# riveSunder/therldaisyworld

Measured on AMD Instinct MI355X. Metric: cell-updates/sec (grid x batch), fused stencil+growth step, higher is better.
Workload: dtype f32

## Files before the change

### therldaisyworld_amd/csrc/dw_api.hip

```cpp
#include <hip/hip_runtime.h>

#include <cmath>
#include <cstdarg>
#include <cstdio>
#include <cstdlib>
#include <cstring>
#include <memory>
#include <new>
#include <type_traits>
#include <vector>

#include "../../include/daisyworld_hip.h"
#include "dw_kernels.hpp"
#include "dw_host_util.hpp"
#include "dw_plan.hpp"
#include "dw_series.hpp"

using namespace dw;

static thread_local char g_err[512] = "";

static int fail(int code, const char* fmt, ...) {
    va_list ap;
    va_start(ap, fmt);
// ... 489 lines not shown
template <class F>
static auto with_fused_layout(const StepPlan& pl, F&& f) {
    if (pl.packed) return f(int_c<kFusedRot>{}, std::true_type{});
    return with_int<kFusedRot, kFusedRing, kFusedOvl>(pl.fused_mode, [&](auto MODE) { return f(MODE, std::false_type{}); });
}

static int launch_forward_fused2(dw_handle* h, double L1, double L2, unsigned int* pstats = nullptr,
                                 float thr_hi = 0.f, StatsDev* trace = nullptr) {
    const dw_params& p = h->prm;
    const StepPlan& pl = h->plan;
    const bool exact = p.precision == DW_PRECISION_EXACT;
    PhysF32 P1, P2;
    if (exact) derive_f32_pair(p, L1, L2, &P1, &P2);
    else { P1 = derive_f32(p, L1); P2 = derive_f32(p, L2); }
    const StepOut o = step_out(h);
    const FusedGeom& g = pl.fgeom;
    const dim3 grid((unsigned)g.chunk * 8u);
    const plane_t *inL = h->L16[h->cur].get(), *inD = h->D16[h->cur].get();
    auto exact_args = [&] {
        return FusedExactArgs{inL, inD, o.L, o.D, g, P1, lum_part(P2), o.zero_me, o.zero_n, pstats, thr_hi, make_f64(p, L1), L1, L2};
    };
    if (trace && exact) {
        const TraceExactArgs A{exact_args(), trace, h->sw.force_rescan ? 1 : 0};
        with_int<kFusedRot, kFusedOvl>(pl.fused_mode, [&](auto MODE) {
            with_bool(pl.sym_albedo, [&](auto SYM) {
                hipLaunchKernelGGL((trace_pair_exact<MODE, SYM>), grid, dim3(256), 0, h->stream, A);
            });
        });
    } else if (trace) {
        with_int<kFusedRot, kFusedOvl>(pl.fused_mode, [&](auto MODE) {
            hipLaunchKernelGGL((trace_pair_fast<MODE>), grid, dim3(256), 0, h->stream, inL, inD, o.L, o.D, g, P1, P2, o.zero_me,
                               o.zero_n, trace);
        });
    } else if (pl.fmt_planes && !pstats && !exact) {
        hipLaunchKernelGGL((step_stream_fused2_fmt_pw<kFusedOvl>), grid, dim3(256), 0, h->stream, inL, inD, o.L, o.D, g, P1, P2,
                           o.zero_me, o.zero_n);
    } else if (exact) {
        const FusedExactArgs A = exact_args();
        with_bool(pstats != nullptr, [&](auto STATS) {
            with_fused_layout(pl, [&](auto MODE, auto PACK) {
                with_bool(pl.sym_albedo, [&](auto SYM) {
                    hipLaunchKernelGGL((step_stream_fused2_exact<MODE, PACK, STATS, SYM>), grid, dim3(256), 0, h->stream, A);
                });
            });
        });
    } else {
        with_bool(pstats != nullptr, [&](auto STATS) {
            with_fused_layout(pl, [&](auto MODE, auto PACK) {
                hipLaunchKernelGGL((step_stream_fused2<MODE, PACK, STATS>), grid, dim3(256), 0, h->stream, inL, inD, o.L, o.D, g,
                                   P1, P2, o.zero_me, o.zero_n, pstats, thr_hi);
            });
        });
    }
    HIPCHK(hipGetLastError());
    step_done(h, L2, false);
    return DW_OK;
}

static int launch_agents(dw_handle* h, const int* d_action, int act_b, int act_n, bool standalone = false,
                         double* d_reward = nullptr, unsigned char* d_done = nullptr, unsigned char* d_ok = nullptr) {
    const dw_params& p = h->prm;
    if (p.n_agents == 0) return DW_OK;
    NEED(h->have_state, DW_ESTATE, "no state uploaded");
    NEED(h->have_agents, DW_ESTATE, "no agents uploaded (call dw_upload_agents or dw_init_random)");
    NEED(p.collision_mode == 0 || standalone, DW_EINVAL,
         "collision_mode=1: call dw_update_agents, apply the collision pass (it consumes the caller's RNG) to the "
// ... 1712 lines not shown
    HIPCHK(hipEventSynchronize(h->ev1));
    HIPCHK(hipEventElapsedTime(elapsed_ms, h->ev0, h->ev1));
    return DW_OK;
}

int dw_device_planes(dw_handle* h, int which, void** light, void** dark) {
    NEED(h && light && dark, DW_EINVAL, "null argument");
    NEED(which == DW_STATE_CURRENT || which == DW_STATE_PREVIOUS, DW_EINVAL, "bad state selector");
    const int buf = which == DW_STATE_CURRENT ? h->cur : 1 - h->cur;
    NEED(which != DW_STATE_CURRENT || cur_quantised(h), DW_ESTATE,
         "the current state is an un-quantised upload: it has no binary16 planes before the first step");
    *light = h->L16[buf].get();
    *dark = h->D16[buf].get();
    return DW_OK;
}

int dw_kernel_info(dw_handle* h, char* buf, size_t buflen) {
    NEED(h && buf && buflen, DW_EINVAL, "null argument");
    const dw_params& p = h->prm;
    const StepPlan& pl = h->plan;
    const char* prec = p.precision == DW_PRECISION_EXACT ? "exact" : (p.precision == DW_PRECISION_FAST ? "fast" : "f64");
    static const char* const halo_name[] = {"rotate", "dpp-old", "general", "packed"};
    if (pl.kind == STEP_STREAM) {
        const StripGeom& g = pl.sgeom;
        snprintf(buf, buflen,
                 "step_stream_%s<halo=%s> wave-strip=%dx256 cells, register window + DPP neighbours, %d-row blocks in "
                 "flight%s, %d strips, grid=%d x 256 threads (4 strips each), XCD-chunked",
                 prec, halo_name[pl.halo], g.SR,
                 p.precision == DW_PRECISION_EXACT ? DW_STREAM_RB_EXACT : DW_STREAM_RB_FAST,
                 p.precision == DW_PRECISION_EXACT ? ", in-wave float64 fix-up from an LDS queue" : "", g.nstrips,
                 g.chunk * 8);
        if (pl.allow_fuse) {
            const size_t n = std::strlen(buf);
            snprintf(buf + n, buflen - n, "; dw_step_n fuses step pairs (step_stream_fused2%s%s)",
                     p.precision == DW_PRECISION_EXACT ? "_exact" : "", pl.fmt_planes ? "_fmt_pw, format buffer accesses" : "");
        }
    } else if (pl.kind == STEP_TILED) {
        const int TR = (256 / pl.tcq) * pl.rpt;
        snprintf(buf, buflen,
                 "step_tiled<TCQ=%d,RPT=%d,%s> tile=%dx%d cells, %zu B LDS/workgroup, %d tiles, grid=%d x 256 threads, "
                 "XCD-chunked",
                 pl.tcq, pl.rpt, prec, TR, pl.tcq * 4, pl.tile_lds, pl.geom.ntiles, pl.geom.chunk * 8);
    } else {
        snprintf(buf, buflen, "step_generic<%s> one thread per cell, grid=(%d,%d) x 256 threads", prec,
                 (p.height * p.width + 255) / 256, p.batch);
    }
    {
        const size_t n = std::strlen(buf);
        snprintf(buf + n, buflen - n, pl.trace_pairs ? "; trace: step pairs" : "; trace: single steps");
    }
    {
        const size_t n = std::strlen(buf);
        snprintf(buf + n, buflen - n, pl.pw_stream ? "; per-world L: wave strips" : "; per-world L: generic");
    }
    {
        static const char* const form_name[] = {"launches per step", "workgroup (LDS)", "one wave per world"};
        const size_t n = std::strlen(buf);
        snprintf(buf + n, buflen - n, "; episode: %s; mlp episode: %s", form_name[episode_form(h)], form_name[episode_mlp_form(h)]);
    }
    {
        const size_t n = std::strlen(buf);
        snprintf(buf + n, buflen - n, "; ensemble episode: %s", ensemble_episode_wave(h) ? "one wave per world" : "launches per step");
    }
    {
        const size_t n = std::strlen(buf);
        snprintf(buf + n, buflen - n, "; episode trace: %s", episode_trace_wave(h) ? "one wave per world" : "launches per step");
    }
    if (pl.first_stream) {
// ... 53 lines not shown
```

### therldaisyworld_amd/csrc/dw_common.hpp

```cpp
#pragma once
#include <type_traits>

#include "dw_physics.hpp"
#include "dw_types.hpp"

namespace dw {

__device__ __forceinline__ float wave_sum(float v) {
#pragma unroll
    for (int o = 32; o > 0; o >>= 1) v += __shfl_xor(v, o, 64);
    return v;
}
__device__ __forceinline__ float wave_max(float v) {
#pragma unroll
    for (int o = 32; o > 0; o >>= 1) v = fmaxf(v, __shfl_xor(v, o, 64));
    return v;
}

__device__ __forceinline__ double to_natural(double x) { return x; }
__device__ __forceinline__ double to_natural(float k) { return (double)k / 1000.0; }
__device__ __forceinline__ double to_natural(plane_t k) { return dw_permille_to_natural((double)(float)k); }
__device__ __forceinline__ float to_permille(double x) { return (float)(x * 1000.0); }
__device__ __forceinline__ float to_permille(float k) { return k; }
__device__ __forceinline__ float to_permille(plane_t k) { return (float)k; }

typedef _Float16 dw_f16x4 __attribute__((ext_vector_type(4)));
typedef unsigned int dw_u32x2 __attribute__((ext_vector_type(2)));
__device__ __forceinline__ dw_f16x4 stream_load4_raw(const plane_t* p) { return *reinterpret_cast<const dw_f16x4*>(p); }
__device__ __forceinline__ float4 widen4(const dw_f16x4& v) { return make_float4((float)v.x, (float)v.y, (float)v.z, (float)v.w); }
__device__ __forceinline__ float4 stream_load4(const plane_t* p) { return widen4(stream_load4_raw(p)); }
__device__ __forceinline__ void stream_store4(plane_t* p, const float4& v) {
    dw_u32x2 t;
    t.x = __builtin_bit_cast(unsigned int, __builtin_amdgcn_cvt_pkrtz(v.x, v.y));
    t.y = __builtin_bit_cast(unsigned int, __builtin_amdgcn_cvt_pkrtz(v.z, v.w));
    __builtin_nontemporal_store(t, reinterpret_cast<dw_u32x2*>(p));
}

typedef float dw_fmt_f32x4 __attribute__((ext_vector_type(4)));
typedef int dw_i32x4 __attribute__((ext_vector_type(4)));
__device__ dw_fmt_f32x4 dw_buf_load_fmt4(dw_i32x4 rsrc, int voff, int soff, int aux) __asm("llvm.amdgcn.raw.buffer.load.format.v4f32");
__device__ void dw_buf_store_fmt4(dw_fmt_f32x4 v, dw_i32x4 rsrc, int voff, int soff, int aux) __asm("llvm.amdgcn.raw.buffer.store.format.v4f32");
constexpr int kBufAuxNonTemporal = 2;
__device__ __forceinline__ dw_i32x4 fmt_plane_rsrc(const plane_t* plane, int world, unsigned int world_bytes) {
    const unsigned long long base = (unsigned long long)plane + (unsigned long long)world * world_bytes;
    dw_i32x4 r;
    r.x = __builtin_amdgcn_readfirstlane((int)(unsigned int)base);
    r.y = __builtin_amdgcn_readfirstlane((int)(unsigned int)(base >> 32)) & 0xffff;
    r.z = __builtin_amdgcn_readfirstlane((int)world_bytes);
    r.w = 0x00067FAC;
    return r;
}
__device__ __forceinline__ float4 fmt_load4(const dw_i32x4& rsrc, int voff, int soff) {
    const dw_fmt_f32x4 v = dw_buf_load_fmt4(rsrc, voff, soff, 0);
    return make_float4(v.x, v.y, v.z, v.w);
}
__device__ __forceinline__ void fmt_store4(const dw_i32x4& rsrc, int voff, int soff, const float4& v) {
    dw_buf_store_fmt4(dw_fmt_f32x4{v.x, v.y, v.z, v.w}, rsrc, voff, soff, kBufAuxNonTemporal);
}
__device__ __forceinline__ float4 widen4(const float4& v) {
    typedef float f2 __attribute__((ext_vector_type(2)));
    unsigned long long lo, hi;
    asm("v_pk_mov_b32 %0, %1, %1 op_sel:[0,1]" : "=v"(lo) : "v"(f2{v.x, v.y}));
    asm("v_pk_mov_b32 %0, %1, %1 op_sel:[0,1]" : "=v"(hi) : "v"(f2{v.z, v.w}));
    return make_float4(__uint_as_float((unsigned int)lo), __uint_as_float((unsigned int)(lo >> 32)),
                       __uint_as_float((unsigned int)hi), __uint_as_float((unsigned int)(hi >> 32)));
}

__device__ __forceinline__ int wrap_near(int v, int n) { return v < 0 ? v + n : (v >= n ? v - n : v); }
__device__ __forceinline__ int wrap_near2(int v, int n) { return wrap_near(wrap_near(v, n), n); }

template <typename T>
__device__ __forceinline__ void gather9(const T* __restrict__ plane, int H, int W, int r, int c,
                                        double out[9]) {
    const int ru = r == 0 ? H - 1 : r - 1, rd = r == H - 1 ? 0 : r + 1;
    const int cl = c == 0 ? W - 1 : c - 1, cr = c == W - 1 ? 0 : c + 1;
    const int rows[3] = {ru, r, rd}, cols[3] = {cl, c, cr};
#pragma unroll
    for (int a = 0; a < 3; ++a)
#pragma unroll
        for (int b = 0; b < 3; ++b) out[a * 3 + b] = to_natural(plane[(size_t)rows[a] * W + cols[b]]);
}

struct Row4 {
    float x[4];
    float h2[4];
};

// ... 55 lines not shown
```

### therldaisyworld_amd/csrc/dw_plan.hpp

```cpp
#pragma once
#include <climits>
#include <cmath>
#include <cstddef>
#include <cstdio>
#include <cstdlib>
#include <cstring>

#include "../../include/daisyworld_hip.h"
#include "dw_types.hpp"

namespace dw {

struct Switches {
    bool no_sym = false, no_pack = false, no_fuse = false, no_ring = false, no_fmt_planes = false, no_episode_kernel = false,
         no_episode_wave = false, no_agent_fuse = false, no_agent_preapply = false, first_f64 = false,
         first_generic = false, force_rescan = false, test_hooks = false;
    int pack_min_strips = -1, strip_rows = 0, tile_rpt = 0, queue_cap = -1, mismatch_cap = -1, trace_rows = 0;
    double first_slack = -1.0;
    char kernel[16] = {0};
    char text[256] = {0};
};
inline const char* test_hook(const char* name) {
    return std::getenv("DW_TEST_HOOKS") ? std::getenv(name) : nullptr;
}
inline Switches read_switches() {
    Switches w;
    auto note = [&](const char* name, const char* val) {
        const size_t n = std::strlen(w.text);
        snprintf(w.text + n, sizeof(w.text) - n, "%s%s%s%s", n ? " " : "", name, val ? "=" : "", val ? val : "");
    };
    auto flag = [&](const char* name, bool& dst) { if (std::getenv(name)) { dst = true; note(name, nullptr); } };
    auto num = [&](const char* name, int& dst, bool test) {
        if (const char* e = test ? test_hook(name) : std::getenv(name)) { dst = std::atoi(e); note(name, e); }
    };
    w.test_hooks = std::getenv("DW_TEST_HOOKS") != nullptr;
    flag("DW_NO_SYM", w.no_sym); flag("DW_NO_PACK", w.no_pack); flag("DW_NO_FUSE", w.no_fuse); flag("DW_NO_RING", w.no_ring);
    flag("DW_NO_FMT_PLANES", w.no_fmt_planes);
    flag("DW_NO_EPISODE_KERNEL", w.no_episode_kernel); flag("DW_NO_EPISODE_WAVE", w.no_episode_wave);
    flag("DW_NO_AGENT_FUSE", w.no_agent_fuse); flag("DW_NO_AGENT_PREAPPLY", w.no_agent_preapply);
    flag("DW_FIRST_STEP_F64", w.first_f64); flag("DW_FIRST_GENERIC", w.first_generic);
    num("DW_PACK_MIN_STRIPS", w.pack_min_strips, false); num("DW_STRIP_ROWS", w.strip_rows, false);
    num("DW_TILE_RPT", w.tile_rpt, false);
    num("DW_TEST_QUEUE_CAP", w.queue_cap, true); num("DW_TEST_MISMATCH_CAP", w.mismatch_cap, true);
    num("DW_TEST_TRACE_ROWS", w.trace_rows, true);
    if (test_hook("DW_TEST_FORCE_RESCAN")) { w.force_rescan = true; note("DW_TEST_FORCE_RESCAN", nullptr); }
    if (const char* e = test_hook("DW_TEST_FIRST_SLACK")) { w.first_slack = std::atof(e); note("DW_TEST_FIRST_SLACK", e); }
    if (const char* e = std::getenv("DW_KERNEL")) { snprintf(w.kernel, sizeof(w.kernel), "%s", e); note("DW_KERNEL", e); }
    return w;
}

inline dw_params with_world_params(dw_params p, const dw_world_params& w) {
    p.p = w.p; p.g = w.g; p.S = w.S; p.sigma = w.sigma; p.gamma = w.gamma; p.q = w.q; p.q2 = w.q2; p.dt = w.dt;
    p.albedo_bare = w.albedo_bare; p.albedo_light = w.albedo_light; p.albedo_dark = w.albedo_dark;
    p.temp_optimal = w.temp_optimal;
    return p;
}
inline dw_world_params world_params_of(const dw_params& p) {
    return dw_world_params{p.p, p.g, p.S, p.sigma, p.gamma, p.q, p.q2, p.dt, p.albedo_bare, p.albedo_light, p.albedo_dark,
                           p.temp_optimal};
}
inline bool albedo_symmetric(double bare, double light, double dark) { return (dark - bare) == -(light - bare); }
inline bool worlds_symmetric(const dw_world_params* worlds, size_t B) {
    for (size_t b = 0; b < B; ++b)
        if (!albedo_symmetric(worlds[b].albedo_bare, worlds[b].albedo_light, worlds[b].albedo_dark)) return false;
    return true;
}

inline PhysF64 make_f64(const dw_params& p, double L) {
    PhysF64 P;
    P.p = p.p; P.g = p.g; P.S = p.S; P.sigma = p.sigma; P.gamma = p.gamma; P.q = p.q; P.q2 = p.q2;
// ... 139 lines not shown
    const double kmax = 1000.0;
    const double a1 = std::fabs((double)P.a1), a2 = std::fabs((double)P.a2), a3 = std::fabs((double)P.a3), a4 = std::fabs((double)P.a4);
    const EConst c0 = e_const(p, L);
    const double c0m = std::fmax(std::fabs(c0.c0l), std::fabs(c0.c0d));
    const double Mmax = (a1 + a2) * 8 * kmax + (a3 + a4) * kmax;
    const double de_max = (8.0 * u + iota) * Mmax + u * c0m;
    const TieChain t = tie_chain(p, c0, P.a1, P.a2, P.a3, P.a4, de_max);
    const double kbe = cbeta_host(p);
    const double Dmin = kbe * (std::sqrt(std::sqrt(t.vlo)) + 1.0) * (std::sqrt(t.vlo) + 1.0);
    const double kK = 5.0 * u + iota;
    const double safety = t.safety, pu = t.pu, kbmax = t.kbmax;
    FirstStepBound B;
    B.a1 = round_up(a1); B.a2 = round_up(a2); B.a3 = round_up(a3); B.a4 = round_up(a4);
    B.c_de = round_up(safety * (8.0 * u + iota) * (1.0 + 8.0 * u));
    B.c_c0 = round_up(safety * u * c0m);
    B.eK0 = round_up(safety * (pu + (kK + 2.0 * u) * std::fabs(p.p) + kbmax * u + ((kK + 3.0 * u) + u) * std::fabs(p.gamma)));
    B.eK1 = round_up(safety * (pu + (kK + 2.0 * u) * std::fabs(p.p) + kbmax * (u + 2.0 * t.ew)));
    B.cW = round_up(safety * 2.0 * kbmax / Dmin);
    B.eA = round_up(safety * ((kK + 3.0 * u) + u + (kK + u)));
    B.cS = round_up(safety * u);
    B.slack = t.admissible ? 4e-6f : 1.0f;
    if (test_slack > (double)B.slack) B.slack = (float)test_slack;
    return B;
}

enum StepKind { STEP_GENERIC, STEP_TILED, STEP_STREAM };
struct StepPlan {
    StepKind kind = STEP_GENERIC;
    int halo = 0;
    bool packed = false;
    bool allow_fuse = false;
    int fused_mode = kFusedOvl;
    bool fmt_planes = false;
    bool trace_pairs = false;
    bool sym_albedo = false;
    int tcq = 0, rpt = 0;
    Geom geom{};
    size_t tile_lds = 0;
    StripGeom sgeom{};
    FusedGeom fgeom{};
    int first_prec = 2;
    bool first_stream = false;
    FirstGeom first_geom{};
    bool need_fixq = false;
    bool pw_stream = false;
};

inline int halo_form(int W) { return W < 256 ? 3 : (W == 256 ? 0 : (W % 256 == 0 ? 1 : 2)); }

inline int strip_rows(long groups, int H, long target) {
    int sr = 64;
    while (sr > 8 && groups * ((H + sr - 1) / sr) < target) sr >>= 1;
    return H < sr ? H : sr;
}

inline int strip_rows_or_override(const Switches& sw, int cap, long groups, int H, long target) {
    if (sw.strip_rows < 1) return strip_rows(groups, H, target);
    const int want = sw.strip_rows < cap ? sw.strip_rows : cap;
    return H < want ? H : want;
}

inline StepPlan plan_steps(const dw_params& p, const Switches& sw) {
    StepPlan s;
    s.sym_albedo = albedo_symmetric(p.albedo_bare, p.albedo_light, p.albedo_dark) && !sw.no_sym;
    s.halo = halo_form(p.width);
    const int lpw = p.width / 4, wpr = lpw ? 64 / lpw : 0;
    const bool pack_shape = p.width >= 8 && p.width < 256 && wpr >= 1 && wpr * lpw * 10 >= 64 * 7 && !sw.no_pack;
    const long pack_strips = pack_shape ? (long)((p.batch + wpr - 1) / wpr) * ((p.height + 63) / 64) : 0;
    const bool packable = pack_shape && pack_strips >= (sw.pack_min_strips >= 0 ? sw.pack_min_strips : 512);
    const bool quads = p.precision != DW_PRECISION_F64 && p.width % 4 == 0;
    if (quads && (p.width >= 256 || packable) && std::strcmp(sw.kernel, "tiled") != 0) {
        s.kind = STEP_STREAM;
        s.packed = p.width < 256;
        StripGeom& g = s.sgeom;
        g.B = p.batch; g.H = p.height; g.W = p.width;
        g.ncs = (p.width + 255) / 256;
        g.lpw = s.packed ? lpw : 64;
        g.wpr = s.packed ? wpr : 1;
        const long groups = s.packed ? (p.batch + wpr - 1) / wpr : p.batch;
        g.SR = strip_rows_or_override(sw, INT_MAX, groups * g.ncs, p.height, 2048);
        g.nrs = (p.height + g.SR - 1) / g.SR;
        g.nstrips = (int)(groups * g.nrs * g.ncs);
        g.nwg = (g.nstrips + 3) / 4;
        g.chunk = (g.nwg + 7) / 8;
        g.qcap = kWaveQueueCap;
        int mcap = kMismatchCap;
        if (sw.queue_cap >= 0 && sw.queue_cap < kWaveQueueCap) g.qcap = sw.queue_cap;
        if (sw.mismatch_cap >= 0 && sw.mismatch_cap < kMismatchCap) mcap = sw.mismatch_cap;
        g.force_rescan = sw.force_rescan ? 1 : 0;
        s.allow_fuse = !sw.no_fuse;
        const bool ring = p.width == 1024 && !sw.no_ring;
        s.fused_mode = p.width <= 256 ? kFusedRot : (ring ? kFusedRing : kFusedOvl);
        FusedGeom& f = s.fgeom;
        f.B = p.batch; f.H = p.height; f.W = p.width;
        f.SR = g.SR;
        f.nrs = g.nrs;
        f.lpw = g.lpw; f.wpr = g.wpr;
        f.cols_per_strip = p.width <= 256 ? 256 : (ring ? 1024 : 248);
        f.ncs = s.packed ? 1 : (p.width + f.cols_per_strip - 1) / f.cols_per_strip;
        f.nstrips = (int)(groups * f.nrs * f.ncs);
        f.nwg = ring ? f.nstrips : (f.nstrips + 3) / 4;
        f.chunk = (f.nwg + 7) / 8;
        f.qcap = g.qcap;
        f.mcap = mcap;
        f.sure_need = 9 * p.n_agents + 9 * mcap + 1;
        s.trace_pairs = s.allow_fuse && !s.packed && s.fused_mode != kFusedRing;
        s.fmt_planes = p.precision == DW_PRECISION_FAST && s.allow_fuse && !s.packed && s.fused_mode == kFusedOvl && !sw.no_fmt_planes &&
                       (size_t)p.height * p.width * sizeof(plane_t) < ((size_t)1 << 31);
    } else if (quads && p.width >= 64) {
        s.kind = STEP_TILED;
        const int Wq = p.width / 4;
        if (Wq >= 64) {
            s.tcq = 64; s.rpt = 4;
            if (sw.tile_rpt == 2 || sw.tile_rpt == 4 || sw.tile_rpt == 8) s.rpt = sw.tile_rpt;
        }
        else if (Wq >= 32) { s.tcq = 32; s.rpt = 4; }
        else { s.tcq = 16; s.rpt = 2; }
        const int TR = (256 / s.tcq) * s.rpt;
        Geom& g = s.geom;
        g.B = p.batch; g.H = p.height; g.W = p.width; g.Wq = Wq;
        g.tiles_r = (p.height + TR - 1) / TR;
        g.tiles_c = (Wq + s.tcq - 1) / s.tcq;
        g.ntiles = p.batch * g.tiles_r * g.tiles_c;
        g.chunk = (g.ntiles + 7) / 8;
        g.qcap = kMaxFix;
        if (sw.queue_cap >= 0 && sw.queue_cap < kMaxFix) g.qcap = sw.queue_cap;
        s.tile_lds = (size_t)2 * (TR + 2) * (s.tcq + 2) * 4 * sizeof(float);
    }
    s.need_fixq = p.precision == DW_PRECISION_EXACT && s.kind == STEP_TILED;
    s.pw_stream = s.kind == STEP_STREAM && !s.packed;
    s.first_prec = p.precision == DW_PRECISION_FAST ? 1 : (p.precision == DW_PRECISION_EXACT && !sw.first_f64 ? 3 : 2);
    s.first_stream = (p.width % 256 == 0 || s.kind == STEP_STREAM) && s.first_prec != 2 && !sw.first_generic;
    if (s.first_stream) {
        FirstGeom& fg = s.first_geom;
        fg.B = p.batch; fg.H = p.height; fg.W = p.width;
        fg.lpw = s.packed ? lpw : 64;
        fg.wpr = s.packed ? wpr : 1;
        fg.ncs = s.packed ? 1 : (p.width + 255) / 256;
        const long groups = s.packed ? (p.batch + fg.wpr - 1) / fg.wpr : p.batch;
        fg.SR = strip_rows_or_override(sw, 64, groups * fg.ncs, p.height, 4096);
        fg.nrs = (p.height + fg.SR - 1) / fg.SR;
// ... 7 lines not shown
```

### therldaisyworld_amd/csrc/dw_step_fused.hpp

```cpp
#pragma once
#include <type_traits>
#include "dw_step_stream.hpp"
#include "dw_types.hpp"

namespace dw {


template <typename TI>
__device__ inline unsigned int exact1_word(const TI* __restrict__ pL, const TI* __restrict__ pD, int H, int W,
                                           int r, int c, const PhysF64& Pa) {
    const int rr = wrap_near2(r, H), cc = wrap_near2(c, W);
    const int ru = rr == 0 ? H - 1 : rr - 1, rd = rr == H - 1 ? 0 : rr + 1;
    const int cl = cc == 0 ? W - 1 : cc - 1, cr = cc == W - 1 ? 0 : cc + 1;
    const int rows[3] = {ru, rr, rd}, cols[3] = {cl, cc, cr};
    unsigned int w1[9];
#pragma unroll
    for (int x = 0; x < 3; ++x)
#pragma unroll
        for (int y = 0; y < 3; ++y) {
            const size_t o = (size_t)rows[x] * W + cols[y];
            w1[x * 3 + y] = (unsigned)(float)pL[o] | ((unsigned)(float)pD[o] << 16);
        }
    const NewCoverF64 s1 = cell_f64_lean(Pa, w1);
    return (unsigned)dw_round3_k(s1.nl) | ((unsigned)dw_round3_k(s1.nd) << 16);
}

template <typename TI>
__device__ inline void exact2_cell(const TI* __restrict__ pL, const TI* __restrict__ pD, int H, int W, int r,
                                   int c, const PhysF64& Pa, const PhysF64& Pb, float& kl, float& kd) {
    unsigned int w2[9];
#pragma unroll
    for (int a = 0; a < 3; ++a)
#pragma unroll
        for (int e = 0; e < 3; ++e) {
            int rr = r + a - 1, cc = c + e - 1;
            rr = rr < 0 ? rr + H : (rr >= H ? rr - H : rr);
            cc = cc < 0 ? cc + W : (cc >= W ? cc - W : cc);
            const int ru = rr == 0 ? H - 1 : rr - 1, rd = rr == H - 1 ? 0 : rr + 1;
            const int cl = cc == 0 ? W - 1 : cc - 1, cr = cc == W - 1 ? 0 : cc + 1;
            const int rows[3] = {ru, rr, rd}, cols[3] = {cl, cc, cr};
            unsigned int w1[9];
#pragma unroll
            for (int x = 0; x < 3; ++x)
#pragma unroll
                for (int y = 0; y < 3; ++y) {
                    const size_t o = (size_t)rows[x] * W + cols[y];
                    w1[x * 3 + y] = (unsigned)(float)pL[o] | ((unsigned)(float)pD[o] << 16);
                }
            const NewCoverF64 s1 = cell_f64_lean(Pa, w1);
            w2[a * 3 + e] = (unsigned)dw_round3_k(s1.nl) | ((unsigned)dw_round3_k(s1.nd) << 16);
        }
    const NewCoverF64 s2 = cell_f64_lean(Pb, w2);
    kl = (float)dw_round3_k(s2.nl);
    kd = (float)dw_round3_k(s2.nd);
}

template <int MODE, bool EXACT, bool PACK = false, bool STATS = false, bool SYM = false, typename TI = plane_t,
          typename TO = plane_t, bool TRACE = false, bool FMT = false>
__device__ __forceinline__ void fused2_body(const TI* __restrict__ inL, const TI* __restrict__ inD,
                                            TO* __restrict__ outL, TO* __restrict__ outD, const FusedGeom& G,
                                            const PhysF32& P1_, const PhysF32& P2_, const PhysF64& P64,
                                            const double& La, const double& Lb,
                                            unsigned long long* __restrict__ zero_me, int zero_n,
                                            unsigned int* __restrict__ pstats = nullptr, float thr_hi = 0.f,
                                            StatsDev* __restrict__ trace = nullptr, int trace_rescan = 0) {
    constexpr bool ROT = MODE == kFusedRot, RING = MODE == kFusedRing;
    static_assert(!RING || !PACK, "the ring exchange is written for un-packed worlds");
    static_assert(!TRACE || (!PACK && !STATS && !RING), "the trace form exists for un-packed overlapped / rotating strips");
    static_assert(!FMT || (MODE == kFusedOvl && !EXACT && !PACK && !STATS && !TRACE), "the format-access form exists for the plain float32 kernel on overlapped strips");
    __shared__ float s_edge[RING ? 2 * 4 * 8 : 1];
    __shared__ uint4 s_queue[EXACT ? 4 * kWaveQueueCap * 3 : 1];
    __shared__ unsigned int s_mm[EXACT ? 4 * kMismatchCap : 1];
    const int bid = blockIdx.x;
    const int wg = (bid & 7) * G.chunk + (bid >> 3);
    if (wg >= G.nwg) return;
    const int tid = threadIdx.x, wv = tid >> 6, lane = tid & 63;
    if (wg == 0)
        for (int i = tid; i < zero_n; i += 256) zero_me[i] = 0ull;
    const int s = RING ? wg : __builtin_amdgcn_readfirstlane(wg * 4 + wv);
    if (!RING && s >= G.nstrips) return;
    uint4* q = s_queue + (EXACT ? wv * kWaveQueueCap * 3 : 0);
    unsigned int* mm = s_mm + (EXACT ? wv * kMismatchCap : 0);
    const int spw = G.nrs * G.ncs;
    const int b = s / spw;
    const int sw = s - b * spw;
    const int rs = sw / G.ncs, cs = sw - rs * G.ncs;
    const int r0 = rs * G.SR;
    const int nr = min(G.SR, G.H - r0);
    const int pw = PACK ? lane / G.lpw : 0, pj = PACK ? lane - pw * G.lpw : 0;
    const int lsrc = PACK ? (pj == 0 ? lane + G.lpw - 1 : lane - 1) : 0;
    const int rsrc = PACK ? (pj == G.lpw - 1 ? lane - (G.lpw - 1) : lane + 1) : 0;
    auto world_off = [&](int lc) -> size_t {
        return (size_t)(PACK ? min(b * G.wpr + min((lc >> 2) / G.lpw, G.wpr - 1), G.B - 1) : b) * G.H * G.W;
    };
    const size_t woff = world_off(4 * lane);
    const int c00 = ROT ? 0 : (RING ? 256 * __builtin_amdgcn_readfirstlane(wv) : cs * 248 - 4);
    int col = PACK ? 4 * pj : c00 + 4 * lane;
    col = col < 0 ? col + G.W : col;
    col = col >= G.W ? col - G.W : col;
    const bool writes = PACK ? (pw < G.wpr && b * G.wpr + pw < G.B)
                             : ((ROT || RING) ? true : (lane >= 1 && lane <= 62 && cs * 248 + 4 * (lane - 1) < G.W));
    bool need1[4] = {true, true, true, true};
    if (PACK) { need1[0] = need1[1] = need1[2] = need1[3] = writes; }
    if (EXACT && !ROT && !RING) {
        const bool wl = __builtin_amdgcn_update_dpp(0, writes ? 1 : 0, kDppWaveShr1, 0xf, 0xf, false) != 0;
        const bool wr = __builtin_amdgcn_update_dpp(0, writes ? 1 : 0, kDppWaveShl1, 0xf, 0xf, false) != 0;
        need1[0] = writes || wl;
        need1[1] = writes;
        need1[2] = writes;
        need1[3] = writes || wr;
    }
    constexpr bool LANE_BOOLS = PACK || (STATS && MODE == kFusedOvl);
    using TieT = std::conditional_t<LANE_BOOLS, bool, unsigned long long>;
    TieT need1m[4], writes_m;
    if constexpr (LANE_BOOLS) {
        for (int i = 0; i < 4; ++i) need1m[i] = need1[i];
        writes_m = writes;
    } else {
        for (int i = 0; i < 4; ++i) need1m[i] = lane_mask(need1[i]);
        writes_m = lane_mask(writes);
    }
    const TI* pL = inL + woff;
    const TI* pD = inD + woff;

    dw_i32x4 fmt_inL, fmt_inD, fmt_outL, fmt_outD;
    int fmt_col = 0, fmt_row = 0;
    if constexpr (FMT) {
        const unsigned int world_bytes = (unsigned int)(G.H * G.W) * 2u;
        fmt_inL = fmt_plane_rsrc(inL, b, world_bytes);
        fmt_inD = fmt_plane_rsrc(inD, b, world_bytes);
        fmt_outL = fmt_plane_rsrc(outL, b, world_bytes);
        fmt_outD = fmt_plane_rsrc(outD, b, world_bytes);
        fmt_col = col * 2;
        fmt_row = G.W * 2;
    }
    struct RawIn { std::conditional_t<FMT, float4, dw_f16x4> l, d; };
    auto load_raw = [&](int rr) -> RawIn {
        rr = min(rr, r0 + nr + 1);
        rr = rr < 0 ? rr + G.H : rr;
        rr = rr >= G.H ? rr - G.H : rr;
        RawIn w;
        if constexpr (FMT) {
            w.l = fmt_load4(fmt_inL, fmt_col, rr * fmt_row);
            w.d = fmt_load4(fmt_inD, fmt_col, rr * fmt_row);
        } else {
            w.l = stream_load4_raw(pL + (size_t)rr * G.W + col);
            w.d = stream_load4_raw(pD + (size_t)rr * G.W + col);
        }
        return w;
    };
    auto pin_edge_sums = [&](Row4& L, Row4& D) {
        asm volatile("" : "+v"(L.h2[0]), "+v"(L.h2[3]), "+v"(D.h2[0]), "+v"(D.h2[3]));
    };
    auto nbrs = [&](const float4& v, float& a, float& c) {
        if (PACK) { a = __shfl(v.w, lsrc, 64); c = __shfl(v.x, rsrc, 64); }
        else if (ROT) { a = dpp_mov_nb<kDppWaveRor1>(v.w); c = dpp_mov_nb<kDppWaveRol1>(v.x); }
        else { a = dpp_mov_nb<kDppWaveShr1>(v.w); c = dpp_mov_nb<kDppWaveShl1>(v.x); }
    };
    auto to_rows4 = [&](const float4& l, const float4& d, Row4& L, Row4& D) {
        float a, c;
        nbrs(l, a, c);
        L = make_row(l, a, c);
        nbrs(d, a, c);
        D = make_row(d, a, c);
    };
    int ring_par = 0;
    auto rows_ring = [&](const float4* v, Row4* const* out, auto NC) {
        constexpr int n = decltype(NC)::value;
        float* mine = s_edge + (ring_par * 4 + wv) * 8;
        if (lane == 63) {
#pragma unroll
            for (int i = 0; i < n; ++i) mine[i] = v[i].w;
        }
        if (lane == 0) {
#pragma unroll
            for (int i = 0; i < n; ++i) mine[4 + i] = v[i].x;
        }
        __syncthreads();
        const float* lw = s_edge + (ring_par * 4 + ((wv + 3) & 3)) * 8;
        const float* rw = s_edge + (ring_par * 4 + ((wv + 1) & 3)) * 8 + 4;
#pragma unroll
        for (int i = 0; i < n; ++i) {
            const float a = dpp_mov<kDppWaveShr1>(lw[i], v[i].w);
            const float c = dpp_mov<kDppWaveShl1>(rw[i], v[i].x);
            *out[i] = make_row(v[i], a, c);
        }
        ring_par ^= 1;
    };
    unsigned int nq = 0;
// ... 194 lines not shown
            Row4* const ob[2] = {&IL[2], &ID[2]};
            rows_ring(va, oa, std::integral_constant<int, 4>{});
            rows_ring(vb, ob, std::integral_constant<int, 2>{});
        } else {
            to_rows4(widen4(p0.l), widen4(p0.d), IL[0], ID[0]);
            to_rows4(widen4(p1.l), widen4(p1.d), IL[1], ID[1]);
            to_rows4(widen4(p2.l), widen4(p2.d), IL[2], ID[2]);
        }
    }
    using U0 = std::integral_constant<int, 0>;
    using U1 = std::integral_constant<int, 1>;
    using U2 = std::integral_constant<int, 2>;
    auto iter = [&](auto U, auto D1, auto D2, int j, auto ST, auto MINE) {
        constexpr int u = decltype(U)::value;
        constexpr bool do1 = decltype(D1)::value, do2 = decltype(D2)::value;
        constexpr bool st_on = STATS && decltype(ST)::value;
        RawIn nx;
        if (do1) nx = load_raw(r0 + j);
        __builtin_amdgcn_sched_barrier(0);
        float l1[4], d1[4], l2[4], d2[4];
        TieT tie1[4], tie2[4];
        float sm1 = 0.f, sm2 = 0.f;
        if (do2)
            row_cells(P2, SL[u], SL[(u + 1) % 3], SL[(u + 2) % 3], SD[u], SD[(u + 1) % 3], SD[(u + 2) % 3], l2, d2, tie2,
                      use2, st_on ? &sm2 : nullptr);
        if (do1)
            row_cells(P1, IL[(u + 2) % 3], IL[u], IL[(u + 1) % 3], ID[(u + 2) % 3], ID[u], ID[(u + 1) % 3], l1, d1, tie1,
                      need1m, st_on ? &sm1 : nullptr);
        if (do2) {
            row_queue(SL[u], SL[(u + 1) % 3], SL[(u + 2) % 3], SD[u], SD[(u + 1) % 3], SD[(u + 2) % 3], l2, d2, tie2, 2,
                      j - 2);
            if (st_on) stats_step2(sm2);
            if constexpr (TRACE) trace_step2(l2, d2);
            if constexpr (FMT) {
                if (writes) {
                    fmt_store4(fmt_outL, fmt_col, (r0 + j - 4) * fmt_row, make_float4(l2[0], l2[1], l2[2], l2[3]));
                    fmt_store4(fmt_outD, fmt_col, (r0 + j - 4) * fmt_row, make_float4(d2[0], d2[1], d2[2], d2[3]));
                }
            } else if (writes) {
                const size_t off = woff + (size_t)(r0 + j - 4) * G.W + col;
                stream_store4(outL + off, make_float4(l2[0], l2[1], l2[2], l2[3]));
                stream_store4(outD + off, make_float4(d2[0], d2[1], d2[2], d2[3]));
            }
        }
        if (do1) {
            row_queue(IL[(u + 2) % 3], IL[u], IL[(u + 1) % 3], ID[(u + 2) % 3], ID[u], ID[(u + 1) % 3], l1, d1, tie1, 1, j);
            if (st_on) stats_step1(sm1, l1, d1, tie1, j >= 2 && j <= nr + 1);
            if constexpr (TRACE) {
                if (decltype(MINE)::value || (j >= 2 && j <= nr + 1)) trace_step1(l1, d1, tie1);
            }
            if constexpr (RING) {
                const float4 v[4] = {make_float4(l1[0], l1[1], l1[2], l1[3]), make_float4(d1[0], d1[1], d1[2], d1[3]),
                                     widen4(nx.l), widen4(nx.d)};
                Row4* const o[4] = {&SL[u], &SD[u], &IL[(u + 2) % 3], &ID[(u + 2) % 3]};
                rows_ring(v, o, std::integral_constant<int, 4>{});
            } else {
                to_rows4(make_float4(l1[0], l1[1], l1[2], l1[3]), make_float4(d1[0], d1[1], d1[2], d1[3]), SL[u], SD[u]);
                __builtin_amdgcn_sched_barrier(0);
                to_rows4(widen4(nx.l), widen4(nx.d), IL[(u + 2) % 3], ID[(u + 2) % 3]);
                if (!PACK) pin_edge_sums(IL[(u + 2) % 3], ID[(u + 2) % 3]);
            }
        }
    };
    using Yes = std::true_type;
    using No = std::false_type;
    iter(U1{}, Yes{}, No{}, 1, Yes{}, No{});
    iter(U2{}, Yes{}, No{}, 2, Yes{}, No{});
// ... 236 lines not shown
        }
    }
}

#ifndef DW_FUSED_FAST_WAVES
#define DW_FUSED_FAST_WAVES 4
#endif
template <int MODE, bool PACK, bool STATS>
constexpr int fused_fast_waves() { return ((MODE == kFusedRing && STATS) || PACK) ? 3 : DW_FUSED_FAST_WAVES; }
template <int MODE, bool PACK = false, bool STATS = false>
__global__ __launch_bounds__(256)
__attribute__((amdgpu_waves_per_eu(fused_fast_waves<MODE, PACK, STATS>(), fused_fast_waves<MODE, PACK, STATS>())))
void step_stream_fused2(const plane_t* __restrict__ inL, const plane_t* __restrict__ inD,
                                                          plane_t* __restrict__ outL, plane_t* __restrict__ outD,
                                                          FusedGeom G, PhysF32 P1, PhysF32 P2,
                                                          unsigned long long* __restrict__ zero_me, int zero_n,
                                                          unsigned int* __restrict__ pstats, float thr_hi) {
    const PhysF64 dummy{};
    const double zero = 0.0;
    fused2_body<MODE, false, PACK, STATS>(inL, inD, outL, outD, G, P1, P2, dummy, zero, zero, zero_me, zero_n, pstats, thr_hi);
}

template <int MODE>
__global__ __launch_bounds__(256) __attribute__((amdgpu_waves_per_eu(DW_FUSED_FAST_WAVES, DW_FUSED_FAST_WAVES)))
void step_stream_fused2_fmt_pw(const plane_t* __restrict__ inL, const plane_t* __restrict__ inD,
                               plane_t* __restrict__ outL, plane_t* __restrict__ outD, FusedGeom G, PhysF32 P1, PhysF32 P2,
                               unsigned long long* __restrict__ zero_me, int zero_n) {
    const PhysF64 dummy{};
    const double zero = 0.0;
    fused2_body<MODE, false, false, false, false, plane_t, plane_t, false, true>(inL, inD, outL, outD, G, P1, P2, dummy, zero,
                                                                                  zero, zero_me, zero_n);
}

#ifndef DW_EXACT_PACK_WAVES
#define DW_EXACT_PACK_WAVES 3
#endif
template <int MODE, bool PACK, bool STATS>
constexpr int fused_exact_waves() {
    return (PACK && STATS) || (STATS && MODE == kFusedRing) ? 2 : (PACK ? DW_EXACT_PACK_WAVES : 3);
}
struct FusedExactArgs {
    const plane_t* inL; const plane_t* inD; plane_t* outL; plane_t* outD;
    FusedGeom G;
    PhysF32 P1; PhysLumF32 lum2;
    unsigned long long* zero_me; int zero_n;
    unsigned int* pstats; float thr_hi;
    PhysF64 P64; double La; double Lb;
};

template <int MODE, bool PACK = false, bool STATS = false, bool SYM = false>
__global__ __launch_bounds__(256)
__attribute__((amdgpu_waves_per_eu(fused_exact_waves<MODE, PACK, STATS>(), fused_exact_waves<MODE, PACK, STATS>())))
void step_stream_fused2_exact(FusedExactArgs A) {
    const FusedExactArgs& cold = kernarg_struct<FusedExactArgs>();
    const PhysF32 P2 = with_lum(A.P1, A.lum2);
    fused2_body<MODE, true, PACK, STATS, SYM>(A.inL, A.inD, A.outL, A.outD, A.G, A.P1, P2, cold.P64, cold.La, cold.Lb, A.zero_me,
                                             A.zero_n, A.pstats, A.thr_hi);
}

#ifndef DW_TRACE_FAST_WAVES
#define DW_TRACE_FAST_WAVES 3
#endif
#ifndef DW_TRACE_EXACT_WAVES
#define DW_TRACE_EXACT_WAVES 2
#endif
template <int MODE>
// ... 28 lines not shown
```

### therldaisyworld_amd/csrc/dw_types.hpp

```cpp
#pragma once

namespace dw {

typedef _Float16 plane_t;

struct PhysF64 {
    double p, g, S, sigma, gamma, q, q2, dt;
    double ab, al, ad, To;
    double L;
    double w0, w1, w2;
};

typedef float dw_f32x2 __attribute__((ext_vector_type(2)));
#define DW_PAIR(lo_name, hi_name, pair_name) \
    union { struct { float lo_name, hi_name; }; dw_f32x2 pair_name; }

struct PhysF32 {
    DW_PAIR(a1h, a2h, a12h);
    DW_PAIR(a3h, a4h, a34h);
    DW_PAIR(a1l, a2l, a12l);
    DW_PAIR(a3l, a4l, a34l);
    DW_PAIR(c0lh, c0ll, c0l);
    DW_PAIR(c0dh, dc0l, c0d);
    DW_PAIR(a1, a2, a12);
// ... 43 lines not shown

struct StripGeom {
    int B, H, W;
    int SR;
    int ncs, nrs;
    int nstrips;
    int nwg;
    int chunk;
    int qcap;
    int lpw, wpr;
    int force_rescan;
};

struct FusedGeom {
    int B, H, W;
    int SR;
    int ncs, nrs;
    int nstrips, nwg, chunk;
    int cols_per_strip;
    int qcap, mcap;
    int lpw, wpr;
    int sure_need;
};

struct FirstGeom {
    int B, H, W;
    int SR;
    int ncs, nrs;
    int nstrips;
    int lpw, wpr;
};

enum { kFusedOvl = 0, kFusedRot = 1, kFusedRing = 2 };
constexpr int kWaveQueueCap = 256;
constexpr int kMismatchCap = 64;
constexpr int kMaxFix = 1024;
constexpr int kNumQueues = 256;

}
```

Before: 787.0 billion.

## Add seam-strip layout: 252-column wave strips with wrapped lane and leftover band kernel

```diff
diff --git a/therldaisyworld_amd/csrc/dw_api.hip b/therldaisyworld_amd/csrc/dw_api.hip
--- a/therldaisyworld_amd/csrc/dw_api.hip
+++ b/therldaisyworld_amd/csrc/dw_api.hip
@@ -545,6 +545,13 @@
             hipLaunchKernelGGL((trace_pair_fast<MODE>), grid, dim3(256), 0, h->stream, inL, inD, o.L, o.D, g, P1, P2, o.zero_me,
                                o.zero_n, trace);
         });
+    } else if (pl.seam_strips && !pstats && !exact) {
+        const FusedGeom &gs = pl.seam_geom, &gl = pl.left_geom;
+        hipLaunchKernelGGL(step_stream_fused2_seam_pw, dim3((unsigned)gs.chunk * 8u), dim3(256), 0, h->stream, inL, inD, o.L, o.D,
+                           gs, P1, P2, o.zero_me, o.zero_n);
+        if (gl.nstrips)
+            hipLaunchKernelGGL(step_stream_fused2_left_pw, dim3((unsigned)gl.chunk * 8u), dim3(256), 0, h->stream, inL, inD, o.L,
+                               o.D, gl, P1, P2, o.zero_me, 0);
     } else if (pl.fmt_planes && !pstats && !exact) {
         hipLaunchKernelGGL((step_stream_fused2_fmt_pw<kFusedOvl>), grid, dim3(256), 0, h->stream, inL, inD, o.L, o.D, g, P1, P2,
                            o.zero_me, o.zero_n);
@@ -2323,8 +2330,16 @@
                  g.chunk * 8);
         if (pl.allow_fuse) {
             const size_t n = std::strlen(buf);
-            snprintf(buf + n, buflen - n, "; dw_step_n fuses step pairs (step_stream_fused2%s%s)",
-                     p.precision == DW_PRECISION_EXACT ? "_exact" : "", pl.fmt_planes ? "_fmt_pw, format buffer accesses" : "");
+            snprintf(buf + n, buflen - n, "; dw_step_n fuses step pairs (step_stream_fused2%s%s",
+                     p.precision == DW_PRECISION_EXACT ? "_exact" : "",
+                     pl.seam_strips ? "_seam_pw, format buffer accesses" : (pl.fmt_planes ? "_fmt_pw, format buffer accesses" : ""));
+            if (pl.seam_strips) {
+                const size_t m = std::strlen(buf);
+                snprintf(buf + m, buflen - m, ", seam strips: %d x %d columns + %d columns of %d row bands per wave", pl.seam_geom.ncs,
+                         kSeamCols, pl.left_geom.cols_per_strip, pl.left_geom.wpr);
+            }
+            const size_t m = std::strlen(buf);
+            snprintf(buf + m, buflen - m, ")");
         }
     } else if (pl.kind == STEP_TILED) {
         const int TR = (256 / pl.tcq) * pl.rpt;
diff --git a/therldaisyworld_amd/csrc/dw_common.hpp b/therldaisyworld_amd/csrc/dw_common.hpp
--- a/therldaisyworld_amd/csrc/dw_common.hpp
+++ b/therldaisyworld_amd/csrc/dw_common.hpp
@@ -39,20 +39,27 @@
 typedef float dw_fmt_f32x4 __attribute__((ext_vector_type(4)));
 typedef int dw_i32x4 __attribute__((ext_vector_type(4)));
 __device__ dw_fmt_f32x4 dw_buf_load_fmt4(dw_i32x4 rsrc, int voff, int soff, int aux) __asm("llvm.amdgcn.raw.buffer.load.format.v4f32");
+__device__ dw_f32x2 dw_buf_load_fmt2(dw_i32x4 rsrc, int voff, int soff, int aux) __asm("llvm.amdgcn.raw.buffer.load.format.v2f32");
 __device__ void dw_buf_store_fmt4(dw_fmt_f32x4 v, dw_i32x4 rsrc, int voff, int soff, int aux) __asm("llvm.amdgcn.raw.buffer.store.format.v4f32");
 constexpr int kBufAuxNonTemporal = 2;
-__device__ __forceinline__ dw_i32x4 fmt_plane_rsrc(const plane_t* plane, int world, unsigned int world_bytes) {
+constexpr int kFmtRsrcQuads = 0x00067FAC, kFmtRsrcPairs = 0x0002FFAC;
+__device__ __forceinline__ dw_i32x4 fmt_plane_rsrc(const plane_t* plane, int world, unsigned int world_bytes,
+                                                   int word3 = kFmtRsrcQuads) {
     const unsigned long long base = (unsigned long long)plane + (unsigned long long)world * world_bytes;
     dw_i32x4 r;
     r.x = __builtin_amdgcn_readfirstlane((int)(unsigned int)base);
     r.y = __builtin_amdgcn_readfirstlane((int)(unsigned int)(base >> 32)) & 0xffff;
     r.z = __builtin_amdgcn_readfirstlane((int)world_bytes);
-    r.w = 0x00067FAC;
+    r.w = word3;
     return r;
 }
 __device__ __forceinline__ float4 fmt_load4(const dw_i32x4& rsrc, int voff, int soff) {
     const dw_fmt_f32x4 v = dw_buf_load_fmt4(rsrc, voff, soff, 0);
     return make_float4(v.x, v.y, v.z, v.w);
+}
+__device__ __forceinline__ float4 fmt_load2x2(const dw_i32x4& rsrc, int voff_a, int voff_b, int soff) {
+    const dw_f32x2 a = dw_buf_load_fmt2(rsrc, voff_a, soff, 0), c = dw_buf_load_fmt2(rsrc, voff_b, soff, 0);
+    return make_float4(a.x, a.y, c.x, c.y);
 }
 __device__ __forceinline__ void fmt_store4(const dw_i32x4& rsrc, int voff, int soff, const float4& v) {
     dw_buf_store_fmt4(dw_fmt_f32x4{v.x, v.y, v.z, v.w}, rsrc, voff, soff, kBufAuxNonTemporal);
diff --git a/therldaisyworld_amd/csrc/dw_plan.hpp b/therldaisyworld_amd/csrc/dw_plan.hpp
--- a/therldaisyworld_amd/csrc/dw_plan.hpp
+++ b/therldaisyworld_amd/csrc/dw_plan.hpp
@@ -12,7 +12,8 @@
 namespace dw {
 
 struct Switches {
-    bool no_sym = false, no_pack = false, no_fuse = false, no_ring = false, no_fmt_planes = false, no_episode_kernel = false,
+    bool no_sym = false, no_pack = false, no_fuse = false, no_ring = false, no_fmt_planes = false, no_seam_strips = false,
+         no_episode_kernel = false,
          no_episode_wave = false, no_agent_fuse = false, no_agent_preapply = false, first_f64 = false,
          first_generic = false, force_rescan = false, test_hooks = false;
     int pack_min_strips = -1, strip_rows = 0, tile_rpt = 0, queue_cap = -1, mismatch_cap = -1, trace_rows = 0;
@@ -35,7 +36,7 @@
     };
     w.test_hooks = std::getenv("DW_TEST_HOOKS") != nullptr;
     flag("DW_NO_SYM", w.no_sym); flag("DW_NO_PACK", w.no_pack); flag("DW_NO_FUSE", w.no_fuse); flag("DW_NO_RING", w.no_ring);
-    flag("DW_NO_FMT_PLANES", w.no_fmt_planes);
+    flag("DW_NO_FMT_PLANES", w.no_fmt_planes); flag("DW_NO_SEAM_STRIPS", w.no_seam_strips);
     flag("DW_NO_EPISODE_KERNEL", w.no_episode_kernel); flag("DW_NO_EPISODE_WAVE", w.no_episode_wave);
     flag("DW_NO_AGENT_FUSE", w.no_agent_fuse); flag("DW_NO_AGENT_PREAPPLY", w.no_agent_preapply);
     flag("DW_FIRST_STEP_F64", w.first_f64); flag("DW_FIRST_GENERIC", w.first_generic);
@@ -241,6 +242,8 @@
     bool allow_fuse = false;
     int fused_mode = kFusedOvl;
     bool fmt_planes = false;
+    bool seam_strips = false;
+    FusedGeom seam_geom{}, left_geom{};
     bool trace_pairs = false;
     bool sym_albedo = false;
     int tcq = 0, rpt = 0;
@@ -267,6 +270,31 @@
     if (sw.strip_rows < 1) return strip_rows(groups, H, target);
     const int want = sw.strip_rows < cap ? sw.strip_rows : cap;
     return H < want ? H : want;
+}
+
+inline long seam_waves_per_world(int W, int nrs) {
+    const int n_full = W / kSeamCols, L = W - kSeamCols * n_full;
+    const int G = L ? 64 / (L / 4 + 2) : 1;
+    return (long)nrs * n_full + (L ? (nrs + G - 1) / G : 0);
+}
+inline bool seam_layout(const FusedGeom& f, FusedGeom* seam, FusedGeom* left) {
+    const int n_full = f.W / kSeamCols, L = f.W - kSeamCols * n_full;
+    if (n_full < 1 || seam_waves_per_world(f.W, f.nrs) >= (long)f.nrs * f.ncs) return false;
+    auto launch = [](FusedGeom& g, long nstrips) {
+        g.nstrips = (int)nstrips;
+        g.nwg = (g.nstrips + 3) / 4;
+        g.chunk = (g.nwg + 7) / 8;
+    };
+    *seam = f;
+    seam->cols_per_strip = kSeamCols;
+    seam->ncs = n_full;
+    launch(*seam, (long)f.B * f.nrs * n_full);
+    *left = *seam;
+    left->cols_per_strip = L;
+    left->lpw = L ? L / 4 + 2 : 64;
+    left->wpr = 64 / left->lpw;
+    launch(*left, L ? (long)f.B * ((f.nrs + left->wpr - 1) / left->wpr) : 0);
+    return true;
 }
 
 inline StepPlan plan_steps(const dw_params& p, const Switches& sw) {
@@ -316,6 +344,7 @@
         s.trace_pairs = s.allow_fuse && !s.packed && s.fused_mode != kFusedRing;
         s.fmt_planes = p.precision == DW_PRECISION_FAST && s.allow_fuse && !s.packed && s.fused_mode == kFusedOvl && !sw.no_fmt_planes &&
                        (size_t)p.height * p.width * sizeof(plane_t) < ((size_t)1 << 31);
+        s.seam_strips = s.fmt_planes && !sw.no_seam_strips && seam_layout(f, &s.seam_geom, &s.left_geom);
     } else if (quads && p.width >= 64) {
         s.kind = STEP_TILED;
         const int Wq = p.width / 4;
diff --git a/therldaisyworld_amd/csrc/dw_step_fused.hpp b/therldaisyworld_amd/csrc/dw_step_fused.hpp
--- a/therldaisyworld_amd/csrc/dw_step_fused.hpp
+++ b/therldaisyworld_amd/csrc/dw_step_fused.hpp
@@ -56,7 +56,7 @@
 }
 
 template <int MODE, bool EXACT, bool PACK = false, bool STATS = false, bool SYM = false, typename TI = plane_t,
-          typename TO = plane_t, bool TRACE = false, bool FMT = false>
+          typename TO = plane_t, bool TRACE = false, bool FMT = false, int SEAM = kSeamNone>
 __device__ __forceinline__ void fused2_body(const TI* __restrict__ inL, const TI* __restrict__ inD,
                                             TO* __restrict__ outL, TO* __restrict__ outD, const FusedGeom& G,
                                             const PhysF32& P1_, const PhysF32& P2_, const PhysF64& P64,
@@ -67,6 +67,7 @@
     constexpr bool ROT = MODE == kFusedRot, RING = MODE == kFusedRing;
     static_assert(!RING || !PACK, "the ring exchange is written for un-packed worlds");
     static_assert(!TRACE || (!PACK && !STATS && !RING), "the trace form exists for un-packed overlapped / rotating strips");
+    static_assert(SEAM == kSeamNone || FMT, "the seam strips exist for the format-access kernel");
     static_assert(!FMT || (MODE == kFusedOvl && !EXACT && !PACK && !STATS && !TRACE), "the format-access form exists for the plain float32 kernel on overlapped strips");
     __shared__ float s_edge[RING ? 2 * 4 * 8 : 1];
     __shared__ uint4 s_queue[EXACT ? 4 * kWaveQueueCap * 3 : 1];
@@ -81,12 +82,17 @@
     if (!RING && s >= G.nstrips) return;
     uint4* q = s_queue + (EXACT ? wv * kWaveQueueCap * 3 : 0);
     unsigned int* mm = s_mm + (EXACT ? wv * kMismatchCap : 0);
-    const int spw = G.nrs * G.ncs;
+    const int spw = SEAM == kSeamLeft ? (G.nrs + G.wpr - 1) / G.wpr : G.nrs * G.ncs;
     const int b = s / spw;
     const int sw = s - b * spw;
-    const int rs = sw / G.ncs, cs = sw - rs * G.ncs;
+    const int rs = SEAM == kSeamLeft ? sw * G.wpr : sw / G.ncs, cs = SEAM == kSeamLeft ? G.ncs : sw - rs * G.ncs;
     const int r0 = rs * G.SR;
     const int nr = min(G.SR, G.H - r0);
+    const int band_g = SEAM == kSeamLeft ? min(lane / G.lpw, G.wpr - 1) : 0;
+    const int band_j = SEAM == kSeamLeft ? min(lane - band_g * G.lpw, G.lpw - 1) : 0;
+    const int band_rs = SEAM == kSeamLeft ? min(rs + band_g, G.nrs - 1) : 0;
+    const int band_dr = SEAM == kSeamLeft ? (band_rs - rs) * G.SR : 0;
+    const int band_nr = SEAM == kSeamLeft ? min(G.SR, G.H - band_rs * G.SR) : 0;
     const int pw = PACK ? lane / G.lpw : 0, pj = PACK ? lane - pw * G.lpw : 0;
     const int lsrc = PACK ? (pj == 0 ? lane + G.lpw - 1 : lane - 1) : 0;
     const int rsrc = PACK ? (pj == G.lpw - 1 ? lane - (G.lpw - 1) : lane + 1) : 0;
@@ -94,11 +100,16 @@
         return (size_t)(PACK ? min(b * G.wpr + min((lc >> 2) / G.lpw, G.wpr - 1), G.B - 1) : b) * G.H * G.W;
     };
     const size_t woff = world_off(4 * lane);
-    const int c00 = ROT ? 0 : (RING ? 256 * __builtin_amdgcn_readfirstlane(wv) : cs * 248 - 4);
-    int col = PACK ? 4 * pj : c00 + 4 * lane;
+    const int c00 = ROT ? 0 : (RING ? 256 * __builtin_amdgcn_readfirstlane(wv)
+                                    : (SEAM == kSeamStrip ? cs * kSeamCols : (SEAM == kSeamLeft ? cs * kSeamCols - 4 : cs * 248 - 4)));
+    int col = PACK ? 4 * pj : c00 + 4 * (SEAM == kSeamLeft ? band_j : lane);
     col = col < 0 ? col + G.W : col;
     col = col >= G.W ? col - G.W : col;
-    const bool writes = PACK ? (pw < G.wpr && b * G.wpr + pw < G.B)
+    int col_b = col + 2;
+    if (SEAM == kSeamStrip && lane == 63) col_b = c00 == 0 ? G.W - 2 : c00 - 2;
+    const bool writes = SEAM == kSeamStrip ? lane < 63
+                      : SEAM == kSeamLeft ? (lane < G.wpr * G.lpw && rs + band_g < G.nrs && band_j >= 1 && band_j <= G.lpw - 2)
+                      : PACK ? (pw < G.wpr && b * G.wpr + pw < G.B)
                              : ((ROT || RING) ? true : (lane >= 1 && lane <= 62 && cs * 248 + 4 * (lane - 1) < G.W));
     bool need1[4] = {true, true, true, true};
     if (PACK) { need1[0] = need1[1] = need1[2] = need1[3] = writes; }
@@ -124,23 +135,35 @@
     const TI* pD = inD + woff;
 
     dw_i32x4 fmt_inL, fmt_inD, fmt_outL, fmt_outD;
-    int fmt_col = 0, fmt_row = 0;
+    int fmt_col = 0, fmt_row = 0, fmt_col_b = 0;
     if constexpr (FMT) {
         const unsigned int world_bytes = (unsigned int)(G.H * G.W) * 2u;
-        fmt_inL = fmt_plane_rsrc(inL, b, world_bytes);
-        fmt_inD = fmt_plane_rsrc(inD, b, world_bytes);
+        fmt_inL = fmt_plane_rsrc(inL, b, world_bytes, SEAM == kSeamStrip ? kFmtRsrcPairs : kFmtRsrcQuads);
+        fmt_inD = fmt_plane_rsrc(inD, b, world_bytes, SEAM == kSeamStrip ? kFmtRsrcPairs : kFmtRsrcQuads);
         fmt_outL = fmt_plane_rsrc(outL, b, world_bytes);
         fmt_outD = fmt_plane_rsrc(outD, b, world_bytes);
         fmt_col = col * 2;
+        fmt_col_b = col_b * 2;
         fmt_row = G.W * 2;
     }
     struct RawIn { std::conditional_t<FMT, float4, dw_f16x4> l, d; };
     auto load_raw = [&](int rr) -> RawIn {
+        RawIn w;
+        if constexpr (SEAM == kSeamLeft) {
+            int lr = min(rr + band_dr, r0 + band_dr + band_nr + 1);
+            lr = lr < 0 ? lr + G.H : lr;
+            lr = lr >= G.H ? lr - G.H : lr;
+            w.l = fmt_load4(fmt_inL, fmt_col + lr * fmt_row, 0);
+            w.d = fmt_load4(fmt_inD, fmt_col + lr * fmt_row, 0);
+            return w;
+        }
         rr = min(rr, r0 + nr + 1);
         rr = rr < 0 ? rr + G.H : rr;
         rr = rr >= G.H ? rr - G.H : rr;
-        RawIn w;
-        if constexpr (FMT) {
+        if constexpr (SEAM == kSeamStrip) {
+            w.l = fmt_load2x2(fmt_inL, fmt_col, fmt_col_b, rr * fmt_row);
+            w.d = fmt_load2x2(fmt_inD, fmt_col, fmt_col_b, rr * fmt_row);
+        } else if constexpr (FMT) {
             w.l = fmt_load4(fmt_inL, fmt_col, rr * fmt_row);
             w.d = fmt_load4(fmt_inD, fmt_col, rr * fmt_row);
         } else {
@@ -154,7 +177,7 @@
     };
     auto nbrs = [&](const float4& v, float& a, float& c) {
         if (PACK) { a = __shfl(v.w, lsrc, 64); c = __shfl(v.x, rsrc, 64); }
-        else if (ROT) { a = dpp_mov_nb<kDppWaveRor1>(v.w); c = dpp_mov_nb<kDppWaveRol1>(v.x); }
+        else if (ROT || SEAM == kSeamStrip) { a = dpp_mov_nb<kDppWaveRor1>(v.w); c = dpp_mov_nb<kDppWaveRol1>(v.x); }
         else { a = dpp_mov_nb<kDppWaveShr1>(v.w); c = dpp_mov_nb<kDppWaveShl1>(v.x); }
     };
     auto to_rows4 = [&](const float4& l, const float4& d, Row4& L, Row4& D) {
@@ -415,7 +438,13 @@
                       j - 2);
             if (st_on) stats_step2(sm2);
             if constexpr (TRACE) trace_step2(l2, d2);
-            if constexpr (FMT) {
+            if constexpr (SEAM == kSeamLeft) {
+                if (writes && j - 4 < band_nr) {
+                    const int voff = fmt_col + (r0 + band_dr + j - 4) * fmt_row;
+                    fmt_store4(fmt_outL, voff, 0, make_float4(l2[0], l2[1], l2[2], l2[3]));
+                    fmt_store4(fmt_outD, voff, 0, make_float4(d2[0], d2[1], d2[2], d2[3]));
+                }
+            } else if constexpr (FMT) {
                 if (writes) {
                     fmt_store4(fmt_outL, fmt_col, (r0 + j - 4) * fmt_row, make_float4(l2[0], l2[1], l2[2], l2[3]));
                     fmt_store4(fmt_outD, fmt_col, (r0 + j - 4) * fmt_row, make_float4(d2[0], d2[1], d2[2], d2[3]));
@@ -718,6 +747,25 @@
                                                                                   zero, zero_me, zero_n);
 }
 
+__global__ __launch_bounds__(256) __attribute__((amdgpu_waves_per_eu(DW_FUSED_FAST_WAVES, DW_FUSED_FAST_WAVES)))
+void step_stream_fused2_seam_pw(const plane_t* __restrict__ inL, const plane_t* __restrict__ inD,
+                                plane_t* __restrict__ outL, plane_t* __restrict__ outD, FusedGeom G, PhysF32 P1, PhysF32 P2,
+                                unsigned long long* __restrict__ zero_me, int zero_n) {
+    const PhysF64 dummy{};
+    const double zero = 0.0;
+    fused2_body<kFusedOvl, false, false, false, false, plane_t, plane_t, false, true, kSeamStrip>(inL, inD, outL, outD, G, P1, P2, dummy,
+                                                                                                 zero, zero, zero_me, zero_n);
+}
+__global__ __launch_bounds__(256) __attribute__((amdgpu_waves_per_eu(DW_FUSED_FAST_WAVES, DW_FUSED_FAST_WAVES)))
+void step_stream_fused2_left_pw(const plane_t* __restrict__ inL, const plane_t* __restrict__ inD,
+                                plane_t* __restrict__ outL, plane_t* __restrict__ outD, FusedGeom G, PhysF32 P1, PhysF32 P2,
+                                unsigned long long* __restrict__ zero_me, int zero_n) {
+    const PhysF64 dummy{};
+    const double zero = 0.0;
+    fused2_body<kFusedOvl, false, false, false, false, plane_t, plane_t, false, true, kSeamLeft>(inL, inD, outL, outD, G, P1, P2, dummy,
+                                                                                                zero, zero, zero_me, zero_n);
+}
+
 #ifndef DW_EXACT_PACK_WAVES
 #define DW_EXACT_PACK_WAVES 3
 #endif
diff --git a/therldaisyworld_amd/csrc/dw_types.hpp b/therldaisyworld_amd/csrc/dw_types.hpp
--- a/therldaisyworld_amd/csrc/dw_types.hpp
+++ b/therldaisyworld_amd/csrc/dw_types.hpp
@@ -99,6 +99,8 @@
 };
 
 enum { kFusedOvl = 0, kFusedRot = 1, kFusedRing = 2 };
+enum { kSeamNone = 0, kSeamStrip = 1, kSeamLeft = 2 };
+constexpr int kSeamCols = 252;
 constexpr int kWaveQueueCap = 256;
 constexpr int kMismatchCap = 64;
 constexpr int kMaxFix = 1024;
```

Result: faster. 800.9 billion, median of 6 (+1.8%).
